# antofuller/jumbo_mae_tpu

Hardware: AMD Instinct MI355X
Metric: pretrain images/sec (whole node) ViT-L/16 224 mask75% at 1/2/4/8 MI355X (higher is better)
Workload: dtype bf16; 1 GPU; model=vit_large_patch16 jumbo-MAE (3 CLS, shared jumbo MLP) + decoder 8x512x16h, global_batch=4096, seq_len=52, decoder_seq_len=199, parallelism=dp1, per_gpu_batch=4096, grad_accum=2, micro_batch=2048, grad_ckpt=False, hip_graph=False, optimizer=adamw(0.9,0.95) wd0.05 warmup-cosine

## Files before the change

### jumbo_mae_tpu_amd/csrc/bindings.cpp

```cpp
#include <torch/extension.h>
#include <c10/hip/HIPStream.h>
#include <hip/hip_runtime.h>

#include <climits>

#include "jm_api.h"

namespace {

hipStream_t stream() { return c10::hip::getCurrentHIPStream().stream(); }

#define CHECK_CUDA(x) TORCH_CHECK((x).is_cuda(), #x " must be a GPU tensor")
#define CHECK_CONTIG(x) TORCH_CHECK((x).is_contiguous(), #x " must be contiguous")
#define CHECK_DT(x, d) TORCH_CHECK((x).scalar_type() == (d), #x " has wrong dtype")

const uint16_t* bf(const torch::Tensor& t) { return reinterpret_cast<const uint16_t*>(t.data_ptr()); }
uint16_t* bfm(torch::Tensor& t) { return reinterpret_cast<uint16_t*>(t.data_ptr()); }
uint16_t* bfp(const torch::Tensor& t) { return reinterpret_cast<uint16_t*>(t.data_ptr()); }
const float* fopt(const c10::optional<torch::Tensor>& t) {
  return t.has_value() && t->defined() ? t->data_ptr<float>() : nullptr;
}
float* fopt_m(c10::optional<torch::Tensor>& t) { return t.has_value() && t->defined() ? t->data_ptr<float>() : nullptr; }

void check_rc(int rc, const char* what) { TORCH_CHECK(rc == 0, what, ": unsupported shape (rc=", rc, ")"); }
// ... 2 lines not shown
  TORCH_CHECK(rate >= 0.0 && rate < 1.0, "dropout rate must be in [0, 1)");
  const double keep = 1.0 - rate;
  return {(uint32_t)std::llround(keep * 65536.0), (float)(1.0 / keep)};
}

static void check_seed(const torch::Tensor& seed, const torch::Tensor& like) {
  TORCH_CHECK(seed.scalar_type() == torch::kInt64 && seed.numel() == 1 && seed.device() == like.device(),
              "dropout seed: int64 [1] on the data's device");
}

JmDrop make_drop(const c10::optional<torch::Tensor>& seed, double rate, const torch::Tensor& like, int64_t ioff) {
  if (!seed.has_value() || !seed->defined() || rate <= 0.0) return JmDrop{nullptr, 0u, 1.f, 0};
  check_seed(*seed, like);
  const auto kp = keep_params(rate);
  return JmDrop{seed->data_ptr<int64_t>(), kp.first, kp.second, (long)ioff};
}

std::vector<torch::Tensor> layernorm_fwd(torch::Tensor x, torch::Tensor gamma, torch::Tensor beta, double eps,
                                         py::object out_dtype, bool also_bf16) {
  CHECK_CUDA(x);
  TORCH_CHECK(x.dim() == 3 && x.stride(2) == 1, "x must be [B,T,D] with contiguous last dim");
  CHECK_DT(x, torch::kFloat32);
  CHECK_CONTIG(gamma);
  CHECK_CONTIG(beta);
  const auto odt = torch::python::detail::py_object_to_dtype(out_dtype);
  const int B = x.size(0), T = x.size(1), D = x.size(2);
  auto y = torch::empty({(long)B * T, D}, x.options().dtype(odt));
  auto mean = torch::empty({(long)B * T}, x.options());
  auto rstd = torch::empty({(long)B * T}, x.options());
  TORCH_CHECK(odt == torch::kBFloat16 || odt == torch::kFloat32, "out dtype must be bf16/fp32");
// ... 74 lines not shown
    CHECK_CONTIG((*hx));
    TORCH_CHECK(hx->numel() == (long)B * T * D, "hx shape");
    TORCH_CHECK(beta.has_value() && beta->defined() && beta->numel() == D, "hx needs beta [D]");
    CHECK_DT((*beta), torch::kFloat32);
    hxp = bf(*hx);
    betap = beta->data_ptr<float>();
  }
  const int NP = has_res ? 4 : 2;
  auto ws = torch::empty({(accum || has_res) ? (long)jm_layernorm_bwd_blocks(B * T, D) * NP * D : 1}, x.options());
  check_rc(jm_layernorm_bwd(dy.data_ptr(), dyb, x.data_ptr<float>(), x.stride(0), x.stride(1), B, T, D,
                            mean.data_ptr<float>(), rstd.data_ptr<float>(), gamma.data_ptr<float>(),
                            dx.data_ptr<float>(), dx.stride(0), dx.stride(1), rp, rB, rT, dgamma.data_ptr<float>(),
                            dbeta.data_ptr<float>(), accum, ws.data_ptr<float>(), has_res ? &res : nullptr,
                            stream(), hxp, betap),
           "layernorm_bwd");
  if (has_res) return {dx, dyr};
  return {dx};
}

torch::Tensor gelu_fwd(torch::Tensor h) {
  CHECK_CONTIG(h);
  CHECK_DT(h, torch::kBFloat16);
  auto a = torch::empty_like(h);
  check_rc(jm_gelu_fwd(bf(h), bfm(a), h.numel(), stream()), "gelu_fwd");
  return a;
}

static torch::Tensor rowcol_ws(const torch::Tensor& like, int M, int N, int nacc) {
  const long n = jm_rowcol_ws_floats(M, N, nacc);
  return torch::empty({n > 0 ? n : 1}, like.options().dtype(torch::kFloat32));
}

torch::Tensor gelu_bwd(torch::Tensor h, torch::Tensor da, c10::optional<torch::Tensor> bias_grad, bool deriv) {
  CHECK_CONTIG(h);
  CHECK_CONTIG(da);
  CHECK_DT(h, torch::kBFloat16);
  CHECK_DT(da, torch::kBFloat16);
  const int N = h.size(-1);
  const int M = h.numel() / N;
  auto dh = torch::empty_like(h);
  float* bg = fopt_m(bias_grad);
  torch::Tensor ws;
  if (bg) ws = rowcol_ws(h, M, N, 1);
  check_rc(jm_gelu_bwd(bf(h), bf(da), bfm(dh), bg, M, N, stream(), deriv ? 1 : 0, bg ? ws.data_ptr<float>() : nullptr),
           "gelu_bwd");
  return dh;
}

void colsum(torch::Tensor x, torch::Tensor acc) {
  CHECK_CONTIG(x);
  CHECK_DT(x, torch::kBFloat16);
  const int N = x.size(-1);
  const int M = x.numel() / N;
  auto ws = rowcol_ws(x, M, N, 1);
  check_rc(jm_colsum_bf16(bf(x), acc.data_ptr<float>(), M, N, stream(), ws.data_ptr<float>()), "colsum");
}

void splitk_reduce_add(torch::Tensor part, torch::Tensor g) {
  CHECK_CONTIG(part);
  TORCH_CHECK(g.is_contiguous() && g.numel() * part.size(0) == part.numel(), "splitk_reduce_add shapes");
  check_rc(jm_splitk_reduce_add(part.data_ptr<float>(), g.data_ptr<float>(), g.numel(), part.size(0), stream()),
           "splitk_reduce_add");
}

void colsum_add_f32(torch::Tensor x, torch::Tensor g) {
  CHECK_CUDA(x);
  CHECK_DT(x, torch::kFloat32);
  CHECK_DT(g, torch::kFloat32);
  TORCH_CHECK(x.dim() == 2 && x.stride(1) == 1 && g.is_contiguous() && g.numel() == x.size(1),
              "colsum_add_f32: x [rows, n] with unit column stride, g [n]");
  TORCH_CHECK(reinterpret_cast<uintptr_t>(x.data_ptr()) % 16 == 0 && reinterpret_cast<uintptr_t>(g.data_ptr()) % 16 == 0,
              "colsum_add_f32: 16-byte aligned operands");
  check_rc(jm_colsum_add_f32(x.data_ptr<float>(), x.stride(0), x.size(0), x.size(1), g.data_ptr<float>(), stream()),
           "colsum_add_f32");
}

torch::Tensor residual_fwd(torch::Tensor x, torch::Tensor y, c10::optional<torch::Tensor> scale,
                           c10::optional<torch::Tensor> mask, c10::optional<torch::Tensor> out_opt,
                           c10::optional<torch::Tensor> seed, double rate, int64_t ioff) {
  TORCH_CHECK(x.dim() == 3 && x.stride(2) == 1, "x must be [B,T,D]");
  CHECK_DT(x, torch::kFloat32);
  CHECK_CONTIG(y);
  CHECK_DT(y, torch::kBFloat16);
  const int B = x.size(0), T = x.size(1), D = x.size(2);
  torch::Tensor out;
  if (out_opt.has_value() && out_opt->defined()) {
    out = *out_opt;
    TORCH_CHECK(out.dim() == 3 && out.size(0) == B && out.size(1) == T && out.size(2) == D && out.stride(2) == 1,
                "out view");
// ... 41 lines not shown
    } else {
      yB = oB;
      yT = oT;
    }
  } else {
    TORCH_CHECK(yB == (long)T * D && yT == D, "residual_bwd: a strided y needs out");
    dy = torch::empty({(long)B * T, D}, dout.options().dtype(odt));
  }
  torch::Tensor ws;
  const bool sums = (dscale && dscale->defined()) || (dbias && dbias->defined());
  if (sums) ws = rowcol_ws(dout, B * T, D, 2);
  check_rc(jm_residual_bwd(dout.data_ptr<float>(), dout.stride(0), dout.stride(1), has_y ? bf(*y) : nullptr,
                           fopt(scale), fopt(mask), fopt_m(dscale), bfm(dy), B, T, D, fopt_m(dbias), yB, yT,
                           stream(), make_drop(seed, rate, dout, ioff), sums ? ws.data_ptr<float>() : nullptr),
           "residual_bwd");
  return dy;
}

static std::tuple<const int64_t*, uint32_t, float> attn_drop(const c10::optional<torch::Tensor>& seed, double rate,
                                                             const torch::Tensor& like) {
  if (!seed.has_value() || !seed->defined() || rate <= 0.0) return {nullptr, 0u, 1.f};
  check_seed(*seed, like);
  const auto kp = keep_params(rate);
  return {seed->data_ptr<int64_t>(), kp.first, kp.second};
}

py::tuple attn_head_dims() {
  const int* d = nullptr;
  const int n = jm_attn_head_dims(&d);
  py::tuple t(n);
// ... 47 lines not shown
             "attn_bwd (long)");
    return dqkv;
  }
  torch::Tensor part;
  const int rows = jm_attn_bwd_part_rows(B, S, hd);
  if (dbias) {
    TORCH_CHECK(dbias->is_contiguous() && dbias->scalar_type() == torch::kFloat32 && dbias->numel() == D3,
                "attn_bwd: dbias must be contiguous fp32 [3D]");
    part = torch::empty({rows, D3}, qkv.options().dtype(torch::kFloat32));
  }
  float* pp = dbias ? part.data_ptr<float>() : nullptr;
  check_rc(jm_attn_bwd(bf(qkv), bf(o), bf(dO), lse.data_ptr<float>(), bfm(dqkv), B, S, heads, hd, pp, std::get<0>(dr),
                       std::get<1>(dr), std::get<2>(dr), stream()),
           "attn_bwd");
  if (dbias) check_rc(jm_splitk_reduce_add(pp, dbias->data_ptr<float>(), D3, rows, stream()), "attn_bwd dbias");
  return dqkv;
}

int nch(const torch::Tensor& chunks) { return chunks.size(0); }
const int* chp(const torch::Tensor& chunks) { return chunks.data_ptr<int>(); }
uint16_t* shadow_ptr(c10::optional<torch::Tensor>& s) {
  return (s.has_value() && s->defined()) ? reinterpret_cast<uint16_t*>(s->data_ptr()) : nullptr;
}

torch::Tensor chunk_part(const torch::Tensor& like, const torch::Tensor& chunks, int nc) {
  return torch::empty({(long)nch(chunks) * nc + 1}, like.options().dtype(torch::kFloat32));
}

void opt_sumsq(torch::Tensor x, torch::Tensor chunks, torch::Tensor out) {
  auto cp = chunk_part(x, chunks, 1);
// ... 322 lines not shown
  torch::Tensor ws;
  const int epi = deriv ? 7 : 2;
  const int r = attach_tail(ep, ws, M, N, K, epi, A);
  int nM = jm_gemm_nt_colpart_rows(M, N, K, epi, A.stride(0));
  if (dbias) {
    TORCH_CHECK(dbias->is_contiguous() && dbias->scalar_type() == torch::kFloat32 && dbias->numel() == N,
                "gemm_nt_dgelu dbias");
    part = r ? torch::zeros({nM + 8 * r, N}, A.options().dtype(torch::kFloat32))
             : torch::empty({nM, N}, A.options().dtype(torch::kFloat32));
    ep.colpart = part.data_ptr<float>();
    nM += 8 * r;
  }
  check_rc(jm_gemm_nt(bf(A), A.stride(0), bf(B), B.stride(0), M, N, K, epi, ep, stream()), "gemm_nt_dgelu");
  if (dbias) check_rc(jm_splitk_reduce_add(part.data_ptr<float>(), dbias->data_ptr<float>(), N, nM, stream()),
                      "gemm_nt_dgelu dbias");
  return out;
}

torch::Tensor rrc_resize(torch::Tensor src, torch::Tensor tab, int64_t size, int64_t tmp_bytes, int64_t tmp_rows_max) {
  CHECK_CUDA(src);
  CHECK_CUDA(tab);
  CHECK_DT(src, torch::kUInt8);
  CHECK_DT(tab, torch::kInt64);
  TORCH_CHECK(src.dim() == 1 && src.is_contiguous(), "rrc_resize: src must be a flat uint8 buffer");
  TORCH_CHECK(tab.dim() == 2 && tab.size(1) == 13 && tab.is_contiguous(), "rrc_resize: tab [B, 13] int64");
  TORCH_CHECK(size > 0 && size <= 4096 && tmp_bytes > 0 && tmp_rows_max > 0, "rrc_resize: bad sizes");
  const int B = tab.size(0);
  auto out = torch::empty({B, 3, size, size}, src.options());
  auto tmp = torch::empty({tmp_bytes}, src.options());
  check_rc(jm_rrc_resize(src.data_ptr<uint8_t>(), tab.data_ptr<int64_t>(), B, (int)size, tmp.data_ptr<uint8_t>(),
// ... 209 lines not shown
  const int sps = jm_gemm_tn_plan(grp, M, &S);
  torch::Tensor part;
  if (S > 1) part = torch::empty({S * total}, gs[0].options());
  int64_t off = 0;
  for (int p = 0; p < np; ++p) {
    grp.out[p] = S > 1 ? part.data_ptr<float>() + off : gs[p].data_ptr<float>();
    off += (int64_t)S * grp.N[p] * grp.K[p];
  }
  const int all_store = group_stores(stores, gs, S, np);
  check_rc(jm_gemm_tn(grp, segmented ? &segs : nullptr, M, sps, S, stream(), all_store), what);
  if (S > 1)
    for (int p = 0; p < np; ++p)
      check_rc(jm_splitk_reduce_add(grp.out[p], gs[p].data_ptr<float>(), (long)grp.N[p] * grp.K[p], S, stream(),
                                    p < (int)stores.size() && stores[p]),
               what);
  return S;
}

int64_t gemm_tn_wgrad(torch::Tensor dy, torch::Tensor x, torch::Tensor g, bool store) {
  return tn_wgrad("gemm_tn_wgrad", {Tensors{dy}}, {Tensors{x}}, {g}, {store}, false);
}

int64_t gemm_tn_wgrad_seg(Tensors dys, Tensors xs, torch::Tensor g, bool store) {
  return tn_wgrad("gemm_tn_wgrad_seg", {dys}, {xs}, {g}, {store}, true);
}

int64_t gemm_tn_wgrad_group(Tensors dys, Tensors xs, Tensors gs, std::vector<bool> stores) {
  std::vector<Tensors> d, x;
  for (const auto& t : dys) d.push_back({t});
  for (const auto& t : xs) x.push_back({t});
// ... 83 lines not shown
  m.def("dropout_apply", &dropout_apply);
  m.def("dropout_apply_", &dropout_apply_);
  m.def("rrc_resize", &rrc_resize, py::arg("src"), py::arg("tab"), py::arg("size"), py::arg("tmp_bytes"),
        py::arg("tmp_rows_max"));
  m.def("rrc_kmax", &jm_rrc_kmax);
  m.def("window_resize", &window_resize, py::arg("src"), py::arg("tab"), py::arg("size"), py::arg("tmp_bytes"),
        py::arg("tmp_rows_max"));
  m.def("window_tab", &jm_window_tab);
  m.def("aug_chain", &aug_chain, py::arg("images"), py::arg("chain"), py::arg("scratch"));
  m.def("gelu_drop", &gelu_drop, py::arg("a"), py::arg("b") = py::none(), py::arg("seed"), py::arg("rate"));
  m.def("softmax_dropout_fwd", &softmax_dropout_fwd);
  m.def("softmax_dropout_bwd", &softmax_dropout_bwd);
  m.def("gelu_bwd", &gelu_bwd, py::arg("h"), py::arg("da"), py::arg("bias_grad") = py::none(),
        py::arg("deriv") = false);
  m.def("colsum", &colsum);
  m.def("splitk_reduce_add", &splitk_reduce_add);
  m.def("residual_ln_fwd", &residual_ln_fwd, py::arg("x"), py::arg("y"), py::arg("scale"), py::arg("mask"),
        py::arg("gamma"), py::arg("beta"), py::arg("eps"), py::arg("T0"), py::arg("R0") = 0,
        py::arg("out") = py::none(), py::arg("seed") = py::none(), py::arg("rate") = 0.0);
  m.def("transpose_bf16", &transpose_bf16);
  m.def("residual_fwd", &residual_fwd, py::arg("x"), py::arg("y"), py::arg("scale"), py::arg("mask"),
        py::arg("out") = py::none(), py::arg("seed") = py::none(), py::arg("rate") = 0.0, py::arg("ioff") = 0);
  m.def("residual_bwd", &residual_bwd, py::arg("dout"), py::arg("y"), py::arg("scale"), py::arg("mask"),
        py::arg("dscale"), py::arg("ydtype"), py::arg("dbias") = py::none(), py::arg("out") = py::none(),
        py::arg("seed") = py::none(), py::arg("rate") = 0.0, py::arg("ioff") = 0);
  m.def("attn_fwd", &attn_fwd, py::arg("qkv"), py::arg("heads"), py::arg("seed") = py::none(), py::arg("rate") = 0.0);
  m.def("attn_bwd", &attn_bwd, py::arg("dO"), py::arg("qkv"), py::arg("o"), py::arg("lse"), py::arg("heads"),
        py::arg("dbias") = py::none(), py::arg("seed") = py::none(), py::arg("rate") = 0.0);
  m.def("attn_max_seq", &jm_attn_max_seq);
  m.def("attn_head_dims", &attn_head_dims);
  m.def("attn_fused_bias", &attn_fused_bias, py::arg("S"), py::arg("hd"));
// ... 58 lines not shown
```

### jumbo_mae_tpu_amd/csrc/elementwise.hip

```cpp
#include "common.h"
#include "jm_api.h"

namespace {

JM_DEVICE float gelu_f(float h) { return gelu_tanh_f(h); }
JM_DEVICE float gelu_grad(float h) { return gelu_grad_f(h); }

__global__ __launch_bounds__(256) void gelu_fwd_kernel(const uint16_t* __restrict__ h, uint16_t* __restrict__ a,
                                                       long n8) {
  for (long i = blockIdx.x * 256L + threadIdx.x; i < n8; i += (long)gridDim.x * 256) {
    float v[8];
    load8(h + i * 8, v);
#pragma unroll
    for (int j = 0; j < 8; ++j) v[j] = gelu_f(v[j]);
    store8(a + i * 8, v);
  }
}

struct ColPlan {
  int cgs, tpr, rps;
};

JM_DEVICE ColPlan col_plan(int N) {
  ColPlan p;
// ... 320 lines not shown
    }
    __syncthreads();
  }
  if (rl == 0 && i < n4) {
    float4* gp = reinterpret_cast<float4*>(g) + i;
    float4 o = store ? make_float4(0.f, 0.f, 0.f, 0.f) : *gp;
    const float4 r = red[c];
    o.x += r.x;
    o.y += r.y;
    o.z += r.z;
    o.w += r.w;
    *gp = o;
  }
}

void launch_colsum(const float* part, float* g, long n4, int S, long ld, int store, hipStream_t st) {
  const long blocks = (n4 + 255) / 256;
  if (blocks >= 512 || S < 16) {
    if (store) jm_zero_f32(g, n4 * 4, st);
    splitk_reduce_add_kernel<<<(unsigned)(blocks > 4096 ? 4096 : blocks), 256, 0, st>>>(part, g, n4, S, ld);
    return;
  }
  int rl = 16;
  while (rl < 256 && S > 32 * rl) rl *= 2;
  const unsigned nb = (unsigned)((n4 * rl + 255) / 256);
  switch (rl) {
    case 16: colsum_rows_kernel<16><<<nb, 256, 0, st>>>(part, g, n4, S, ld, store); break;
    case 32: colsum_rows_kernel<32><<<nb, 256, 0, st>>>(part, g, n4, S, ld, store); break;
    case 64: colsum_rows_kernel<64><<<nb, 256, 0, st>>>(part, g, n4, S, ld, store); break;
    case 128: colsum_rows_kernel<128><<<nb, 256, 0, st>>>(part, g, n4, S, ld, store); break;
    default: colsum_rows_kernel<256><<<nb, 256, 0, st>>>(part, g, n4, S, ld, store); break;
// ... 23 lines not shown
  for (long i = (long)blockIdx.x * 256 + threadIdx.x; i < n; i += (long)gridDim.x * 256) p[i] = 0.f;
}
}

void jm_zero_f32(float* p, long n, hipStream_t st) {
  if (n <= 0) return;
  long blocks = (n + 255) / 256;
  if (blocks > 2048) blocks = 2048;
  zero_f32_kernel<<<(unsigned)blocks, 256, 0, st>>>(p, n);
}

int jm_splitk_reduce_add(const float* part, float* g, long n, int S, hipStream_t st, int store) {
  if (n % 4) return -1;
  const long n4 = n / 4;
  if (S >= 1 && S <= 16 && n4 >= 256L * 256) {
    const unsigned nb = (unsigned)((n4 + 255) / 256);
    switch (S) {
#define JM_SKR(SS)                                                                     \
  case SS:                                                                             \
    if (store) splitk_reduce_add_s_kernel<SS, true><<<nb, 256, 0, st>>>(part, g, n4);  \
    else splitk_reduce_add_s_kernel<SS><<<nb, 256, 0, st>>>(part, g, n4);              \
    return 0;
      JM_SKR(1) JM_SKR(2) JM_SKR(3) JM_SKR(4) JM_SKR(5) JM_SKR(6) JM_SKR(7) JM_SKR(8)
      JM_SKR(9) JM_SKR(10) JM_SKR(11) JM_SKR(12) JM_SKR(13) JM_SKR(14) JM_SKR(15) JM_SKR(16)
#undef JM_SKR
      default: break;
    }
  }
  launch_colsum(part, g, n4, S, n, store, st);
  return 0;
}

int jm_colsum_add_f32(const float* x, long ld, int rows, long n, float* g, hipStream_t st) {
  if (n % 4 || ld % 4 || ld < n || rows < 1) return -1;
  launch_colsum(x, g, n / 4, rows, ld, 0, st);
  return 0;
}

namespace {
__global__ __launch_bounds__(256) void zero_ranges_kernel(float* __restrict__ base, const long long* __restrict__ desc,
                                                          int n) {
  long long b = blockIdx.x;
  int r = 0;
  for (; r < n; ++r) {
    const long long nb = (desc[2 * r + 1] + 4095) / 4096;
// ... 229 lines not shown
```

### jumbo_mae_tpu_amd/csrc/jm_api.h

```cpp
#pragma once
#include <cstddef>
#include <cstdint>

#include <hip/hip_runtime.h>

struct JmDrop {
  const int64_t* seed;
  uint32_t thr;
  float scale;
  long ioff;
};

struct JmLnRes {
  const uint16_t* y;
  uint16_t* dy;
  long yB, yT;
  const float* scale;
  const float* mask;
  int T0;
  float* dscale;
  float* dbias;
  JmDrop drop;
};

// ... 23 lines not shown
  float* colpart;
  float* part;
  int splits;
  float* tail;
  int tail_S;
  int t_begin;
  int t_count;
  const int64_t* dseed;
  uint32_t dthr;
  float dscale;
  uint8_t* dq;
  const uint8_t* dqa;
  float dqs;
};


int jm_layernorm_fwd(const float* x, long sB, long sT, int B, int T, int D, const float* gamma, const float* beta,
                     float eps, void* y, int out_bf16, float* mean, float* rstd, hipStream_t st, uint16_t* y2 = nullptr);
int jm_layernorm_bwd(const void* dy, int dy_bf16, const float* x, long sB, long sT, int B, int T, int D,
                     const float* mean, const float* rstd, const float* gamma, float* dx_ptr, long oB, long oT,
                     const float* dres, long rB, long rT, float* dgamma, float* dbeta, int accum_params, float* ws,
                     const JmLnRes* res, hipStream_t st, const uint16_t* hx = nullptr,
                     const float* beta = nullptr);
int jm_layernorm_bwd_blocks(int rows, int D);
int jm_residual_ln_fwd(const float* x, long sB, long sT, const uint16_t* y, const float* scale, const float* mask,
                       float* x1, long oB, long oT, uint16_t* h, float* mean, float* rstd, int B, int T, int T0,
                       int D, const float* gamma, const float* beta, float eps, hipStream_t st, int R0 = 0,
                       JmDrop drop = JmDrop{nullptr, 0u, 1.f, 0});
int jm_debug_line_layernorm();

int jm_gelu_fwd(const uint16_t* h, uint16_t* a, long n, hipStream_t st);
long jm_rowcol_ws_floats(int M, int N, int nacc);
int jm_gelu_bwd(const uint16_t* h, const uint16_t* da, uint16_t* dh, float* bias_grad, int M, int N, hipStream_t st,
                int deriv, float* ws);
int jm_colsum_bf16(const uint16_t* x, float* acc, int M, int N, hipStream_t st, float* ws);
int jm_residual_fwd(const float* x, long sB, long sT, int B, int T, int D, const uint16_t* y, const float* scale,
                    const float* mask, float* out, long oB, long oT, hipStream_t st, JmDrop drop);
int jm_residual_bwd(const float* dout, long dB, long dT, const uint16_t* y, const float* scale, const float* mask,
                    float* dscale, uint16_t* dy, int B, int T, int D, float* dbias, long yB, long yT, hipStream_t st,
                    JmDrop drop, float* ws);
void jm_zero_f32(float* p, long n, hipStream_t st);
int jm_splitk_reduce_add(const float* part, float* g, long n, int S, hipStream_t st, int store = 0);
int jm_colsum_add_f32(const float* x, long ld, int rows, long n, float* g, hipStream_t st);
int jm_zero_ranges(float* base, const long long* desc, int n, long long blocks, hipStream_t st);
int jm_transpose_bf16(const uint16_t* src, uint16_t* dst, int R, int C, hipStream_t st);
int jm_transpose_bf16_batch(const long long* desc, int n, int tiles, hipStream_t st);
int jm_splitk_reduce_bf16(const float* part, int S, long n, int N, const float* bias, uint16_t* out, hipStream_t st);
int jm_splitk_reduce_f32(const float* part, int S, int M, int N, const float* bias, const float* add, long add_ld,
                         float* out, hipStream_t st);
int jm_debug_line_elementwise();
void jm_debug_selftest(int v, hipStream_t st);

int jm_attn_fwd(const uint16_t* qkv, uint16_t* o, float* lse, int B, int S, int H, int hd, const int64_t* dseed,
                uint32_t dthr, float dscale, hipStream_t st);
int jm_attn_bwd(const uint16_t* qkv, const uint16_t* o, const uint16_t* dO, const float* lse, uint16_t* dqkv, int B,
                int S, int H, int hd, float* dbias_part, const int64_t* dseed, uint32_t dthr, float dscale,
                hipStream_t st);
// ... 83 lines not shown
```

### jumbo_mae_tpu_amd/csrc/layernorm.hip

```cpp
#include <type_traits>

#include "common.h"
#include "jm_api.h"

namespace {

template <int V, typename TO>
__global__ __launch_bounds__(256) void ln_fwd_kernel(const float* __restrict__ x, long sB, long sT, int T,
                                                     int rows, int D, const float* __restrict__ gamma,
                                                     const float* __restrict__ beta, float eps,
                                                     TO* __restrict__ y, float* __restrict__ mean_out,
                                                     float* __restrict__ rstd_out, uint16_t* __restrict__ y2) {
  const int wave = threadIdx.x >> 6, lane = threadIdx.x & 63;
  const int row = blockIdx.x * 4 + wave;
  if (row >= rows) return;
  const int b = row / T, t = row - b * T;
  const float* xr = x + b * sB + t * sT;
  float v[V][4];
  float s = 0.f;
#pragma unroll
  for (int i = 0; i < V; ++i) {
    const int col = (i * 64 + lane) * 4;
    if (col < D) {
      load4(xr + col, v[i]);
// ... 398 lines not shown
    __syncthreads();
  }
  if (rl == 0 && i4 < n4) {
    const float4 r = red[c];
    const float v[4] = {r.x, r.y, r.z, r.w};
#pragma unroll
    for (int j = 0; j < 4; ++j) {
      const int col = i4 * 4 + j;
      float* dst = outs.p[col / D];
      if (dst != nullptr) dst[col % D] += v[j];
    }
  }
}

void launch_param_reduce(const float* ws, int nb, int D, int NP, ParamOuts outs, hipStream_t st) {
  int rl = 16;
  while (rl < 256 && nb > 32 * rl) rl *= 2;
  const unsigned grid = (unsigned)((NP * D / 4) * rl + 255) / 256;
  switch (rl) {
    case 16: ln_param_reduce_kernel<16><<<grid, 256, 0, st>>>(ws, nb, D, NP, outs); break;
    case 32: ln_param_reduce_kernel<32><<<grid, 256, 0, st>>>(ws, nb, D, NP, outs); break;
    case 64: ln_param_reduce_kernel<64><<<grid, 256, 0, st>>>(ws, nb, D, NP, outs); break;
    case 128: ln_param_reduce_kernel<128><<<grid, 256, 0, st>>>(ws, nb, D, NP, outs); break;
    default: ln_param_reduce_kernel<256><<<grid, 256, 0, st>>>(ws, nb, D, NP, outs); break;
  }
}

template <typename TO>
void launch_fwd(int V, dim3 grid, hipStream_t st, const float* x, long sB, long sT, int T, int rows, int D,
                const float* g, const float* b, float eps, TO* y, float* m, float* r, uint16_t* y2) {
// ... 210 lines not shown
                       int D, const float* gamma, const float* beta, float eps, hipStream_t st, int R0,
                       JmDrop drop) {
  const ResLnIO io{x, sB, sT, y, scale, mask, x1, oB, oT, h, mean, rstd, drop};
  if (R0 < 0 || R0 >= T) return -2;
  const int V = pick_v(D);
  if (V < 0 || (D % 4) != 0) return -1;
  const int rows = B * T;
  dim3 grid((rows + 3) / 4);
#define JM_RLN(VV) \
  case VV: res_ln_fwd_kernel<VV><<<grid, 256, 0, st>>>(io, T, T0, R0, rows, D, gamma, beta, eps); break;
  switch (V) {
    JM_RLN(1) JM_RLN(2) JM_RLN(3) JM_RLN(4) JM_RLN(6) JM_RLN(8) JM_RLN(9) JM_RLN(12) JM_RLN(16)
    default: return -1;
  }
#undef JM_RLN
  return 0;
}

constexpr int LN_BWD_CUS = 256;
int ln_bwd_blocks_per_cu(int V) { return V <= 1 ? 4 : V <= 4 ? 3 : 2; }

int jm_layernorm_bwd_blocks(int rows, int D) {
  if (use_wide(rows, D)) return rows > 1024 ? 1024 : rows;
  const int V = pick_v(D), cap = LN_BWD_CUS * ln_bwd_blocks_per_cu(V < 0 ? 16 : V);
  const int rpb = 4 * LN_BWD_R(V);
  int nb = (rows + rpb - 1) / rpb;
  return nb > cap ? cap : nb;
}

int jm_layernorm_bwd(const void* dy, int dy_bf16, const float* x, long sB, long sT, int B, int T, int D,
// ... 65 lines not shown
```

### jumbo_mae_tpu_amd/ops/blocks.py

```python

from __future__ import annotations


import torch

from typing import NamedTuple

from . import dropout as Dr
from . import prims as P


LINKS = True
FWD_LINKS = True


class Link:

    __slots__ = ("spec", "dy", "done", "dx_key", "ln1", "h1")

    def __init__(self, ln1=None):
        self.spec = None
        self.dy = None
        self.done = False
        self.dx_key = None
# ... 107 lines not shown
        else:
            P.residual_fwd(pin, fy, layer.scale2, m2, out=x2[:, C:], drop=_od(dr, "fo", fy))
        ctx.save_for_backward(x, mu1, rs1, h1, qkv, o, lse, a, x1, muc, rsc, hcb, jpre, jg, jy,
                              hp, mup, rsp, fpre, fg, fy, m1, m2, m3)
        ctx.layer = layer
        ctx.link_in, ctx.link_out = link_in, link_out
        ctx.gelu_deriv = (jd, fd)
        ctx.gelu_rate = rate
        ctx.dr = dr
        if link_out is not None:
            link_out.spec = P.ResSpec(fy, layer.scale2, m2, layer.ff.w2.b, C, drop=_od(dr, "fo", fy))
        return x2

    @staticmethod
    def backward(ctx, dx2):
        with P.paired_wgrads():
            dx = _jumbo_bwd(ctx, dx2)
        return dx, None, None, None, None, None, None, None, None, None


def _jumbo_bwd(ctx, dx2):
    (x, mu1, rs1, h1, qkv, o, lse, a, x1, muc, rsc, hcb, jpre, jg, jy,
     hp, mup, rsp, fpre, fg, fy, m1, m2, m3) = ctx.saved_tensors
    layer = ctx.layer
    dr = ctx.dr
    B, S, D = x.shape
    C = layer.C
    J = C * D
    dt = h1.dtype
    dx2 = dx2.contiguous()
    dx1 = torch.empty_like(dx2)
# ... 66 lines not shown
            link_out.put_h1(x2, h1n, mun, rsn)
        else:
            x2 = P.residual_fwd(x1, fy, layer.scale2, m2, drop=_od(dr, "fo", fy))
        ctx.save_for_backward(x, mu1, rs1, h1, qkv, o, lse, a, x1, mu2, rs2, h2, fpre, fg, fy, m1, m2)
        ctx.layer = layer
        ctx.link_in, ctx.link_out = link_in, link_out
        ctx.gelu_deriv = (False, fd)
        ctx.gelu_rate = dr.rate if dr is not None else 0.0
        ctx.dr = dr
        if link_out is not None:
            link_out.spec = P.ResSpec(fy, layer.scale2, m2, layer.ff.w2.b, 0, drop=_od(dr, "fo", fy))
        return x2

    @staticmethod
    def backward(ctx, dx2):
        with P.paired_wgrads():
            dx = _vit_bwd(ctx, dx2)
        return dx, None, None, None, None, None, None, None, None


def _vit_bwd(ctx, dx2):
    x, mu1, rs1, h1, qkv, o, lse, a, x1, mu2, rs2, h2, fpre, fg, fy, m1, m2 = ctx.saved_tensors
    layer = ctx.layer
    dr = ctx.dr
    B, S, D = x.shape
    dt = h1.dtype
    dx2 = dx2.contiguous()
    fused = ctx.link_out.take(dx2) if ctx.link_out is not None else None
    if fused is not None:
        dfy, bd = fused
    else:
# ... 15 lines not shown
```

### jumbo_mae_tpu_amd/ops/prims.py

```python

from __future__ import annotations

import contextlib
import math
import os

from typing import NamedTuple

import torch
import torch.nn.functional as F

from ..models.params import Handle
from . import _ext

LN_EPS = 1e-6
_GELU_C = math.sqrt(2.0 / math.pi)


def hip(t: torch.Tensor) -> bool:
    return _ext.use_hip(t)


def _trainable(h: Handle | None) -> bool:
    return h is not None and h.segs[0].trainable
# ... 37 lines not shown
            part = torch.bmm(dy.view(s, M // s, N).transpose(1, 2), x.view(s, M // s, K), out_dtype=torch.float32)
            if hip(part):
                _ext.load().splitk_reduce_add(part, g)
            else:
                g.add_(part.sum(0))
        else:
            torch.addmm(g, dy.t(), x, out_dtype=torch.float32, out=g)
    else:
        g.addmm_(dy.t().float(), x.float())


PAIR_WGRAD = True
_pair: dict = {"depth": 0, "held": None}


@contextlib.contextmanager
def paired_wgrads():
    _pair["depth"] += 1
    try:
        yield
    finally:
        _pair["depth"] -= 1
        if _pair["depth"] == 0:
            _flush_pair()


def _flush_pair() -> None:
    held, _pair["held"] = _pair["held"], None
    if held is not None:
        hw, dy, x = held
        wgrad(hw, dy, x)
        hw.ready()


def _wgrad_ready(hw: Handle, dy: torch.Tensor, x: torch.Tensor) -> None:
    if PAIR_WGRAD and _pair["depth"] > 0 and _tn_ok(dy, x):
        held = _pair["held"]
        if held is not None and held[1].shape[0] == dy.shape[0] and held[0] is not hw:
            _pair["held"] = None
            _ext.load().gemm_tn_wgrad_group([held[1], dy], [held[2], x], [held[0].grad, hw.grad],
                                            [held[0].take_store(), hw.take_store()])
            held[0].ready()
            hw.ready()
            return
        _flush_pair()
        _pair["held"] = (hw, dy, x)
        return
    wgrad(hw, dy, x)
    hw.ready()


def bias_grad(hb: Handle, dy: torch.Tensor) -> None:
    if hip(dy) and dy.dtype == torch.bfloat16 and dy.shape[-1] % 8 == 0 and dy.stride(-1) == 1:
        _ext.load().colsum(dy, hb.grad)
    else:
        hb.grad.add_(dy.sum(0, dtype=torch.float32))


_GEMM_MODE = "auto"
_DGRAD_OURS = True


NARROW_MAX_M = 4096
_NARROW_FUSED_MIN_TILES = 160
# ... 117 lines not shown

def _flush_seg_group(todo: list) -> list:
    if not GROUP_JUMBO_WGRAD or len(todo) != 2:
        return todo
    (h1, p1), (h2, p2) = todo
    if any(h.store.partial_hooks and len(h.segs) == 1 for h in (h1, h2)) or len(p1) != len(p2):
        return todo
    d1, x1 = [p[0] for p in p1], [p[1] for p in p1]
    d2, x2 = [p[0] for p in p2], [p[1] for p in p2]
    if not (_seg_ok(d1, x1) and _seg_ok(d2, x2) and d1[0].shape[0] == d2[0].shape[0]
            and d1[0].shape[0] % 64 == 0 and h1.grad.is_contiguous() and h2.grad.is_contiguous()):
        return todo
    _ext.load().gemm_tn_wgrad_seg_group([d1, d2], [x1, x2], [h1.grad, h2.grad], [h1.take_store(), h2.take_store()])
    for h, pairs in todo:
        for _ in pairs:
            h.ready()
    return []


def flush_deferred_wgrads() -> None:
    _deferred["cb"] = False
    hs, _deferred["handles"] = _deferred["handles"], []
    todo = []
    for h in hs:
        pairs, h.deferred = h.deferred, []
        if pairs:
            todo.append((h, pairs))
    for h, pairs in _flush_seg_group(todo):
        dys = [p[0] for p in pairs]
        xs = [p[1] for p in pairs]
        N, K = dys[0].shape[1], xs[0].shape[1]
# ... 5 lines not shown
            dy = torch.cat(dys) if len(dys) > 1 else dys[0]
            x = torch.cat(xs) if len(xs) > 1 else xs[0]
        store = h.take_store() if seg else False
        if len(chunks) > 1 and not seg:
            h.settle()
        for r0, r1 in chunks:
            if seg:
                _ext.load().gemm_tn_wgrad_seg([d[:, r0:r1] for d in dys], xs, h.grad[r0:r1], store)
            elif len(chunks) == 1:
                wgrad(h, dy, x)
            else:
                wgrad(h, dy[:, r0:r1], x, rows=(r0, r1))
            if len(chunks) > 1:
                h.store.mark_partial_ready(h, r0 * K, r1 * K)
        for _ in pairs:
            h.ready()


def _defer_wgrad(hw: Handle, dy: torch.Tensor, x2: torch.Tensor) -> bool:
    if not _deferred["cb"]:
        try:
            torch.autograd.Variable._execution_engine.queue_callback(flush_deferred_wgrads)
        except RuntimeError:
            return False
        _deferred["cb"] = True
    if not hw.deferred:
        _deferred["handles"].append(hw)
    hw.deferred.append((dy, x2))
    return True


# ... 34 lines not shown
        return _ext.load().gemm_nt(dy.contiguous(), hw.weight_t(), None, False)[0]
    if (_DGRAD_OURS and hip(dy) and dy.dtype == torch.bfloat16 and w.shape[0] % 64
            and use_our_gemm(dy.shape[0], w.shape[1], -(-w.shape[0] // 64) * 64, kind="dgrad")):
        return _ext.load().gemm_nt(_pad_cols(dy), _pad_cols(hw.weight_t()), None, False)[0]
    return dy @ w


def linear_bwd(dy: torch.Tensor, x2: torch.Tensor, hw: Handle, hb: Handle | None, need_dx: bool = True,
               bias_done: bool = False, dx_add: torch.Tensor | None = None):
    dx = linear_dgrad(dy, hw, dx_add) if need_dx else None
    if (_trainable(hw) and hw.defer_wgrad and _deferred["enabled"] and (hip(dy) or _deferred["force"])
            and _defer_wgrad(hw, dy, x2)):
        if hb is not None:
            if not bias_done:
                bias_grad(hb, dy)
            hb.ready()
        return dx
    if _trainable(hw):
        side = wgrad_stream() if dy.is_cuda else None
        if side is not None:
            if not _side["cb"]:
                torch.autograd.Variable._execution_engine.queue_callback(_end_of_backward)
                _side["cb"] = True
            side.wait_stream(torch.cuda.current_stream())
            with torch.cuda.stream(side):
                wgrad(hw, dy, x2)
                if hb is not None and not bias_done:
                    bias_grad(hb, dy)
            dy.record_stream(side)
            x2.record_stream(side)
            hw.ready()
        else:
            if hb is not None and not bias_done:
                bias_grad(hb, dy)
            _wgrad_ready(hw, dy, x2)
        if hb is not None:
            hb.ready()
    return dx


def linear_gelu_bwd(dy: torch.Tensor, g: torch.Tensor, pre: torch.Tensor, hw2: Handle, hb2: Handle | None,
                    hb1: Handle | None, bias2_done: bool = False, deriv: bool = False, rate: float = 0.0):
    w2 = hw2.weight()
    M, N, K = dy.shape[0], w2.shape[1], w2.shape[0]
    if (_DGRAD_OURS and hip(dy) and dy.dtype == torch.bfloat16 and N % 8 == 0
            and (not deriv or pre.dtype == torch.uint8)
            and use_our_gemm(M, N, K, fused_gelu=True, kind="dgrad")):
        bg = hb1.grad if _trainable(hb1) else None
        dpre = _ext.load().gemm_nt_dgelu(dy.contiguous(), hw2.weight_t(), pre.contiguous(), bg, deriv, rate)
        linear_bwd(dy, g, hw2, hb2, need_dx=False, bias_done=bias2_done)
        return dpre, bg is not None
    if deriv and pre.dtype == torch.uint8:
# ... 93 lines not shown
        xf = x3.reshape(B * T, D).float()
        xhat = (xf - mean[:, None]) * rstd[:, None]
        dyf = dy.reshape(B * T, D).float()
        if tr:
            hg.grad.add_((dyf * xhat).sum(0))
            hb.grad.add_(dyf.sum(0))
        g = dyf * hg.master
        dx = rstd[:, None] * (g - g.mean(-1, keepdim=True) - xhat * (g * xhat).mean(-1, keepdim=True))
        dx = dx.reshape(B, T, D)
        if dres is not None:
            dx = dx + dres
        if out is not None:
            out.copy_(dx)
            dx = out
    if tr:
        hg.ready()
        hb.ready()
    if res is None:
        return dx
    if fused:
        if _trainable(res.hs):
            res.hs.ready()
        return dx, dyr, _trainable(res.hbias)
    dyr, done = residual_bwd(dx[:, res.t0:], res.y, res.hs, res.mask, res.y.dtype, res.hbias, out=res.out,
                             drop=res.drop)
    return dx, dyr, done


def residual_fwd(x3: torch.Tensor, y2: torch.Tensor, hs: Handle | None, mask, out=None, drop=None) -> torch.Tensor:
    B, T, D = x3.shape
    if hip(x3):
        y2r = y2.reshape(B * T, D)
        dseed, drate, dioff = _drop_args(y2r, drop)
        return _ext.load().residual_fwd(x3, y2r, hs.master if hs is not None else None, mask, out, dseed, drate,
                                        dioff)
    r = y2.float()
    if drop is not None:
# ... 45 lines not shown
            d = d * mask.view(B, 1, 1)
        if drop is not None:
            d = d * _drop_factor(y2, drop).reshape(B, T, D)
        if hs is not None:
            if _trainable(hs):
                hs.grad.add_((d * y2.float().reshape(B, T, D)).sum((0, 1)))
            d = d * hs.master
        dy = d.to(ydtype)
        if out is not None:
            out.copy_(dy.reshape(out.shape))
            dy = out
        else:
            dy = dy.reshape(B * T, D)
        done = False
    if mark_ready and _trainable(hs):
        hs.ready()
    return dy, done


def _attn_hip(qkv: torch.Tensor, heads: int) -> bool:
    if not hip(qkv):
        return False
    hd = qkv.shape[2] // 3 // heads
    return hd in _ext.load().attn_head_dims()


_ATTN_DROP_TILED = True


def _attn_drop_hip(S: int, hd: int) -> bool:
    ext = _ext.load()
# ... 57 lines not shown
```

Measured before the change: 6664 images/sec.

## Group small gradient reductions per block backward into one batched launch

Adds a grouped-reduction scope that queues the small parameter-gradient reductions issued during each transformer block's backward (LayerNorm param partials, bias colsums, split-K partial sums) and launches them together as one kernel with a job table, instead of one launch each. Workspaces are kept alive until the flush, and handle ready() calls are deferred until the group closes. The aim is to cut kernel-launch overhead and tail underutilisation from many tiny reductions. In exchange, gradient readiness for overlapping communication or optimizer work is delayed to the end of each block, and there is new bookkeeping for aliasing and stream consistency.

Result: no change. 6684 images/sec (median of 6 runs) (+0.3%).

```diff
diff --git a/jumbo_mae_tpu_amd/csrc/bindings.cpp b/jumbo_mae_tpu_amd/csrc/bindings.cpp
--- a/jumbo_mae_tpu_amd/csrc/bindings.cpp
+++ b/jumbo_mae_tpu_amd/csrc/bindings.cpp
@@ -40,6 +40,21 @@
   check_seed(*seed, like);
   const auto kp = keep_params(rate);
   return JmDrop{seed->data_ptr<int64_t>(), kp.first, kp.second, (long)ioff};
+}
+
+thread_local std::vector<torch::Tensor> rg_held;
+
+void rg_keep(const torch::Tensor& t) {
+  if (t.defined() && jm_rg_pending() > 0) rg_held.push_back(t);
+}
+
+void rg_begin(bool slices) { jm_rg_begin(slices ? 1 : 0); }
+
+int64_t rg_pending() { return jm_rg_pending(); }
+
+void rg_end() {
+  jm_rg_end(stream());
+  if (jm_rg_pending() == 0) rg_held.clear();
 }
 
 std::vector<torch::Tensor> layernorm_fwd(torch::Tensor x, torch::Tensor gamma, torch::Tensor beta, double eps,
@@ -144,6 +159,7 @@
                             dbeta.data_ptr<float>(), accum, ws.data_ptr<float>(), has_res ? &res : nullptr,
                             stream(), hxp, betap),
            "layernorm_bwd");
+  rg_keep(ws);
   if (has_res) return {dx, dyr};
   return {dx};
 }
@@ -174,6 +190,7 @@
   if (bg) ws = rowcol_ws(h, M, N, 1);
   check_rc(jm_gelu_bwd(bf(h), bf(da), bfm(dh), bg, M, N, stream(), deriv ? 1 : 0, bg ? ws.data_ptr<float>() : nullptr),
            "gelu_bwd");
+  rg_keep(ws);
   return dh;
 }
 
@@ -184,13 +201,35 @@
   const int M = x.numel() / N;
   auto ws = rowcol_ws(x, M, N, 1);
   check_rc(jm_colsum_bf16(bf(x), acc.data_ptr<float>(), M, N, stream(), ws.data_ptr<float>()), "colsum");
-}
-
-void splitk_reduce_add(torch::Tensor part, torch::Tensor g) {
+  rg_keep(ws);
+}
+
+void splitk_reduce_add(torch::Tensor part, torch::Tensor g, bool store) {
   CHECK_CONTIG(part);
   TORCH_CHECK(g.is_contiguous() && g.numel() * part.size(0) == part.numel(), "splitk_reduce_add shapes");
-  check_rc(jm_splitk_reduce_add(part.data_ptr<float>(), g.data_ptr<float>(), g.numel(), part.size(0), stream()),
+  check_rc(jm_splitk_reduce_add(part.data_ptr<float>(), g.data_ptr<float>(), g.numel(), part.size(0), stream(),
+                                store ? 1 : 0),
            "splitk_reduce_add");
+  rg_keep(part);
+}
+
+void ln_param_reduce(torch::Tensor ws, std::vector<c10::optional<torch::Tensor>> outs) {
+  CHECK_CUDA(ws);
+  CHECK_CONTIG(ws);
+  CHECK_DT(ws, torch::kFloat32);
+  const int NP = (int)outs.size();
+  TORCH_CHECK(ws.dim() == 2 && NP >= 1 && NP <= 4 && ws.size(1) % NP == 0, "ln_param_reduce: ws [nb, NP * D], NP <= 4");
+  const int D = ws.size(1) / NP;
+  float* po[4] = {nullptr, nullptr, nullptr, nullptr};
+  for (int k = 0; k < NP; ++k) {
+    if (!outs[k].has_value() || !outs[k]->defined()) continue;
+    TORCH_CHECK(outs[k]->is_contiguous() && outs[k]->scalar_type() == torch::kFloat32 && outs[k]->numel() == D &&
+                    outs[k]->device() == ws.device(),
+                "ln_param_reduce: outputs fp32 [D] on ws's device");
+    po[k] = outs[k]->data_ptr<float>();
+  }
+  check_rc(jm_ln_param_reduce(ws.data_ptr<float>(), (int)ws.size(0), D, NP, po, stream()), "ln_param_reduce");
+  rg_keep(ws);
 }
 
 void colsum_add_f32(torch::Tensor x, torch::Tensor g) {
@@ -203,6 +242,7 @@
               "colsum_add_f32: 16-byte aligned operands");
   check_rc(jm_colsum_add_f32(x.data_ptr<float>(), x.stride(0), x.size(0), x.size(1), g.data_ptr<float>(), stream()),
            "colsum_add_f32");
+  rg_keep(x);
 }
 
 torch::Tensor residual_fwd(torch::Tensor x, torch::Tensor y, c10::optional<torch::Tensor> scale,
@@ -274,6 +314,7 @@
                            fopt(scale), fopt(mask), fopt_m(dscale), bfm(dy), B, T, D, fopt_m(dbias), yB, yT,
                            stream(), make_drop(seed, rate, dout, ioff), sums ? ws.data_ptr<float>() : nullptr),
            "residual_bwd");
+  rg_keep(ws);
   return dy;
 }
 
@@ -351,6 +392,7 @@
                        std::get<1>(dr), std::get<2>(dr), stream()),
            "attn_bwd");
   if (dbias) check_rc(jm_splitk_reduce_add(pp, dbias->data_ptr<float>(), D3, rows, stream()), "attn_bwd dbias");
+  rg_keep(part);
   return dqkv;
 }
 
@@ -703,6 +745,7 @@
   check_rc(jm_gemm_nt(bf(A), A.stride(0), bf(B), B.stride(0), M, N, K, epi, ep, stream()), "gemm_nt_dgelu");
   if (dbias) check_rc(jm_splitk_reduce_add(part.data_ptr<float>(), dbias->data_ptr<float>(), N, nM, stream()),
                       "gemm_nt_dgelu dbias");
+  rg_keep(part);
   return out;
 }
 
@@ -942,6 +985,7 @@
       check_rc(jm_splitk_reduce_add(grp.out[p], gs[p].data_ptr<float>(), (long)grp.N[p] * grp.K[p], S, stream(),
                                     p < (int)stores.size() && stores[p]),
                what);
+  rg_keep(part);
   return S;
 }
 
@@ -1055,7 +1099,13 @@
   m.def("gelu_bwd", &gelu_bwd, py::arg("h"), py::arg("da"), py::arg("bias_grad") = py::none(),
         py::arg("deriv") = false);
   m.def("colsum", &colsum);
-  m.def("splitk_reduce_add", &splitk_reduce_add);
+  m.def("splitk_reduce_add", &splitk_reduce_add, py::arg("part"), py::arg("g"), py::arg("store") = false);
+  m.def("ln_param_reduce", &ln_param_reduce, "the LayerNorm backward's parameter-partial reduction alone");
+  m.def("rg_begin", &rg_begin, py::arg("slices") = false,
+        "open a grouped-reduction scope: the small gradient reductions issued until the matching rg_end run as one "
+        "launch there (slices: the weight gradients' split-K slice sums too)");
+  m.def("rg_end", &rg_end, "close the scope; the outermost one launches what is queued on the current stream");
+  m.def("rg_pending", &rg_pending, "queued reduction jobs");
   m.def("residual_ln_fwd", &residual_ln_fwd, py::arg("x"), py::arg("y"), py::arg("scale"), py::arg("mask"),
         py::arg("gamma"), py::arg("beta"), py::arg("eps"), py::arg("T0"), py::arg("R0") = 0,
         py::arg("out") = py::none(), py::arg("seed") = py::none(), py::arg("rate") = 0.0);
diff --git a/jumbo_mae_tpu_amd/csrc/elementwise.hip b/jumbo_mae_tpu_amd/csrc/elementwise.hip
--- a/jumbo_mae_tpu_amd/csrc/elementwise.hip
+++ b/jumbo_mae_tpu_amd/csrc/elementwise.hip
@@ -358,7 +358,181 @@
   }
 }
 
+namespace rg {
+__device__ __forceinline__ void rows_job(const RgJob& j, int lb, float4* red) {
+  const int RL = j.rl, CW = 256 / RL;
+  const int c = threadIdx.x % CW, rl = threadIdx.x / CW;
+  const long i = lb * (long)CW + c;
+  const int S = j.S;
+  float4 acc = make_float4(0.f, 0.f, 0.f, 0.f);
+  if (i < j.n4) {
+    const float4* p = reinterpret_cast<const float4*>(j.src) + i;
+    const long l4 = j.ld / 4;
+    int s = rl;
+    for (; s + 3 * RL < S; s += 4 * RL) {
+      const float4 a = p[(long)s * l4], b = p[(long)(s + RL) * l4];
+      const float4 e = p[(long)(s + 2 * RL) * l4], f = p[(long)(s + 3 * RL) * l4];
+      acc.x += (a.x + b.x) + (e.x + f.x);
+      acc.y += (a.y + b.y) + (e.y + f.y);
+      acc.z += (a.z + b.z) + (e.z + f.z);
+      acc.w += (a.w + b.w) + (e.w + f.w);
+    }
+    for (; s < S; s += RL) {
+      const float4 a = p[(long)s * l4];
+      acc.x += a.x;
+      acc.y += a.y;
+      acc.z += a.z;
+      acc.w += a.w;
+    }
+  }
+  red[threadIdx.x] = acc;
+  __syncthreads();
+  for (int h = RL / 2; h >= 1; h >>= 1) {
+    if (rl < h) {
+      const float4 o = red[threadIdx.x + h * CW];
+      float4& r = red[threadIdx.x];
+      r.x += o.x;
+      r.y += o.y;
+      r.z += o.z;
+      r.w += o.w;
+    }
+    __syncthreads();
+  }
+  if (rl == 0 && i < j.n4) {
+    float4* gp = reinterpret_cast<float4*>(j.dst) + i;
+    float4 o = j.store ? make_float4(0.f, 0.f, 0.f, 0.f) : *gp;
+    const float4 r = red[c];
+    o.x += r.x;
+    o.y += r.y;
+    o.z += r.z;
+    o.w += r.w;
+    *gp = o;
+  }
+}
+
+__device__ __forceinline__ void seq_job(const RgJob& j, int lb) {
+  const long i = lb * 256L + threadIdx.x;
+  if (i >= j.n4) return;
+  const long n = j.ld;
+  const int S = j.S;
+  float acc[4] = {0.f, 0.f, 0.f, 0.f};
+  int s = 0;
+  for (; s + 1 < S; s += 2) {
+    float v[4], w[4];
+    load4(j.src + (long)s * n + i * 4, v);
+    load4(j.src + (long)(s + 1) * n + i * 4, w);
+#pragma unroll
+    for (int k = 0; k < 4; ++k) acc[k] += v[k] + w[k];
+  }
+  if (s < S) {
+    float v[4];
+    load4(j.src + (long)s * n + i * 4, v);
+#pragma unroll
+    for (int k = 0; k < 4; ++k) acc[k] += v[k];
+  }
+  float o[4] = {0.f, 0.f, 0.f, 0.f};
+  if (!j.store) load4(j.dst + i * 4, o);
+#pragma unroll
+  for (int k = 0; k < 4; ++k) o[k] += acc[k];
+  store4(j.dst + i * 4, o);
+}
+
+__device__ __forceinline__ void slices_job(const RgJob& j, int lb) {
+  const long i = lb * 256L + threadIdx.x;
+  if (i >= j.n4) return;
+  const long n = j.ld;
+  const int S = j.S;
+  float o[4] = {0.f, 0.f, 0.f, 0.f};
+  if (!j.store) load4(j.dst + i * 4, o);
+  int s = 0;
+  for (; s + 3 < S; s += 4) {
+    float v[4][4];
+#pragma unroll
+    for (int u = 0; u < 4; ++u) load4(j.src + (long)(s + u) * n + i * 4, v[u]);
+#pragma unroll
+    for (int u = 0; u < 4; ++u)
+#pragma unroll
+      for (int k = 0; k < 4; ++k) o[k] += v[u][k];
+  }
+  for (; s < S; ++s) {
+    float v[4];
+    load4(j.src + (long)s * n + i * 4, v);
+#pragma unroll
+    for (int k = 0; k < 4; ++k) o[k] += v[k];
+  }
+  store4(j.dst + i * 4, o);
+}
+
+__global__ __launch_bounds__(256) void reduce_group_kernel(const RgTable tab) {
+  __shared__ float4 red[256];
+  const int b = blockIdx.x;
+  int lo = 0, hi = tab.n - 1;
+  while (lo < hi) {
+    const int mid = (lo + hi + 1) >> 1;
+    if (tab.job[mid].block0 <= b) lo = mid;
+    else hi = mid - 1;
+  }
+  const RgJob j = tab.job[lo];
+  const int lb = b - j.block0;
+  if (j.kind == RG_ROWS) rows_job(j, lb, red);
+  else if (j.kind == RG_SEQ) seq_job(j, lb);
+  else slices_job(j, lb);
+}
+
+struct Queue {
+  RgTable tab;
+  int depth = 0;
+  int slices = 0;
+  hipStream_t st = nullptr;
+};
+thread_local Queue q;
+
+void launch(hipStream_t st) {
+  if (q.tab.n == 0) return;
+  reduce_group_kernel<<<(unsigned)q.tab.blocks, 256, 0, st>>>(q.tab);
+  q.tab.n = 0;
+  q.tab.blocks = 0;
+}
+
+void push(RgJob j, long blocks, hipStream_t st) {
+  bool clash = q.tab.n == RG_MAX_JOBS || q.tab.blocks + blocks > (1L << 30);
+  for (int i = 0; i < q.tab.n && !clash; ++i) {
+    const RgJob& o = q.tab.job[i];
+    clash = j.dst < o.dst + o.n4 * 4 && o.dst < j.dst + j.n4 * 4;
+  }
+  if (clash) launch(q.st);
+  j.block0 = q.tab.blocks;
+  q.tab.job[q.tab.n++] = j;
+  q.tab.blocks += (int)blocks;
+  q.st = st;
+}
+
+bool open(hipStream_t st) { return q.depth > 0 && (q.tab.n == 0 || q.st == st); }
+
+bool aligned16(const void* p) { return reinterpret_cast<uintptr_t>(p) % 16 == 0; }
+
+int colsum_rl(int S) {
+  int rl = 16;
+  while (rl < 256 && S > 32 * rl) rl *= 2;
+  return rl;
+}
+
+void push_colsum(const float* part, float* g, long n4, int S, long ld, int store, bool rows, hipStream_t st) {
+  const long blocks = (n4 + 255) / 256;
+  if (!rows && (blocks >= 512 || S < 16)) {
+    push(RgJob{part, g, ld, n4, S, RG_SEQ, 0, store, 0}, blocks, st);
+    return;
+  }
+  const int rl = colsum_rl(S);
+  push(RgJob{part, g, ld, n4, S, RG_ROWS, rl, store, 0}, (n4 * rl + 255) / 256, st);
+}
+}
+
 void launch_colsum(const float* part, float* g, long n4, int S, long ld, int store, hipStream_t st) {
+  if (rg::open(st) && ld % 4 == 0 && rg::aligned16(part) && rg::aligned16(g)) {
+    rg::push_colsum(part, g, n4, S, ld, store, false, st);
+    return;
+  }
   const long blocks = (n4 + 255) / 256;
   if (blocks >= 512 || S < 16) {
     if (store) jm_zero_f32(g, n4 * 4, st);
@@ -412,6 +586,10 @@
   if (n % 4) return -1;
   const long n4 = n / 4;
   if (S >= 1 && S <= 16 && n4 >= 256L * 256) {
+    if (rg::q.slices && rg::open(st)) {
+      rg::push(RgJob{part, g, n, n4, S, RG_SLICES, 0, store, 0}, (n4 + 255) / 256, st);
+      return 0;
+    }
     const unsigned nb = (unsigned)((n4 + 255) / 256);
     switch (S) {
 #define JM_SKR(SS)                                                                     \
@@ -427,6 +605,27 @@
   }
   launch_colsum(part, g, n4, S, n, store, st);
   return 0;
+}
+
+void jm_rg_begin(int slices) {
+  if (rg::q.depth++ == 0) rg::q.slices = slices;
+}
+
+int jm_rg_pending() { return rg::q.tab.n; }
+
+void jm_rg_flush(hipStream_t st) { rg::launch(rg::q.tab.n ? rg::q.st : st); }
+
+void jm_rg_end(hipStream_t st) {
+  if (rg::q.depth > 0 && --rg::q.depth == 0) jm_rg_flush(st);
+}
+
+int jm_rg_ln_params(const float* ws, int nb, int D, int NP, float* const* outs, hipStream_t st) {
+  if (!rg::open(st) || D % 4 || !rg::aligned16(ws)) return 0;
+  for (int k = 0; k < NP; ++k)
+    if (outs[k] && !rg::aligned16(outs[k])) return 0;
+  for (int k = 0; k < NP; ++k)
+    if (outs[k]) rg::push_colsum(ws + (long)k * D, outs[k], D / 4, nb, (long)NP * D, 0, true, st);
+  return 1;
 }
 
 int jm_colsum_add_f32(const float* x, long ld, int rows, long n, float* g, hipStream_t st) {
diff --git a/jumbo_mae_tpu_amd/csrc/jm_api.h b/jumbo_mae_tpu_amd/csrc/jm_api.h
--- a/jumbo_mae_tpu_amd/csrc/jm_api.h
+++ b/jumbo_mae_tpu_amd/csrc/jm_api.h
@@ -61,6 +61,25 @@
   float dqs;
 };
 
+enum { RG_ROWS = 0, RG_SEQ = 1, RG_SLICES = 2 };
+struct RgJob {
+  const float* src;
+  float* dst;
+  long ld;
+  long n4;
+  int S;
+  int kind;
+  int rl;
+  int store;
+  int block0;
+};
+constexpr int RG_MAX_JOBS = 64;
+struct RgTable {
+  RgJob job[RG_MAX_JOBS];
+  int n;
+  int blocks;
+};
+
 
 int jm_layernorm_fwd(const float* x, long sB, long sT, int B, int T, int D, const float* gamma, const float* beta,
                      float eps, void* y, int out_bf16, float* mean, float* rstd, hipStream_t st, uint16_t* y2 = nullptr);
@@ -69,6 +88,7 @@
                      const float* dres, long rB, long rT, float* dgamma, float* dbeta, int accum_params, float* ws,
                      const JmLnRes* res, hipStream_t st, const uint16_t* hx = nullptr,
                      const float* beta = nullptr);
+int jm_ln_param_reduce(const float* ws, int nb, int D, int NP, float* const* outs, hipStream_t st);
 int jm_layernorm_bwd_blocks(int rows, int D);
 int jm_residual_ln_fwd(const float* x, long sB, long sT, const uint16_t* y, const float* scale, const float* mask,
                        float* x1, long oB, long oT, uint16_t* h, float* mean, float* rstd, int B, int T, int T0,
@@ -88,6 +108,11 @@
                     JmDrop drop, float* ws);
 void jm_zero_f32(float* p, long n, hipStream_t st);
 int jm_splitk_reduce_add(const float* part, float* g, long n, int S, hipStream_t st, int store = 0);
+void jm_rg_begin(int slices);
+void jm_rg_end(hipStream_t st);
+void jm_rg_flush(hipStream_t st);
+int jm_rg_pending();
+int jm_rg_ln_params(const float* ws, int nb, int D, int NP, float* const* outs, hipStream_t st);
 int jm_colsum_add_f32(const float* x, long ld, int rows, long n, float* g, hipStream_t st);
 int jm_zero_ranges(float* base, const long long* desc, int n, long long blocks, hipStream_t st);
 int jm_transpose_bf16(const uint16_t* src, uint16_t* dst, int R, int C, hipStream_t st);
diff --git a/jumbo_mae_tpu_amd/csrc/layernorm.hip b/jumbo_mae_tpu_amd/csrc/layernorm.hip
--- a/jumbo_mae_tpu_amd/csrc/layernorm.hip
+++ b/jumbo_mae_tpu_amd/csrc/layernorm.hip
@@ -436,6 +436,7 @@
 }
 
 void launch_param_reduce(const float* ws, int nb, int D, int NP, ParamOuts outs, hipStream_t st) {
+  if (jm_rg_ln_params(ws, nb, D, NP, outs.p, st)) return;
   int rl = 16;
   while (rl < 256 && nb > 32 * rl) rl *= 2;
   const unsigned grid = (unsigned)((NP * D / 4) * rl + 255) / 256;
@@ -676,6 +677,14 @@
     default: return -1;
   }
 #undef JM_RLN
+  return 0;
+}
+
+int jm_ln_param_reduce(const float* ws, int nb, int D, int NP, float* const* outs, hipStream_t st) {
+  if (D % 4 || NP < 1 || NP > 4 || nb < 1) return -1;
+  ParamOuts po{{nullptr, nullptr, nullptr, nullptr}};
+  for (int k = 0; k < NP; ++k) po.p[k] = outs[k];
+  launch_param_reduce(ws, nb, D, NP, po, st);
   return 0;
 }
 
diff --git a/jumbo_mae_tpu_amd/ops/blocks.py b/jumbo_mae_tpu_amd/ops/blocks.py
--- a/jumbo_mae_tpu_amd/ops/blocks.py
+++ b/jumbo_mae_tpu_amd/ops/blocks.py
@@ -145,7 +145,7 @@
 
     @staticmethod
     def backward(ctx, dx2):
-        with P.paired_wgrads():
+        with P.paired_wgrads(P.hip(dx2)):
             dx = _jumbo_bwd(ctx, dx2)
         return dx, None, None, None, None, None, None, None, None, None
 
@@ -242,7 +242,7 @@
 
     @staticmethod
     def backward(ctx, dx2):
-        with P.paired_wgrads():
+        with P.paired_wgrads(P.hip(dx2)):
             dx = _vit_bwd(ctx, dx2)
         return dx, None, None, None, None, None, None, None, None
 
diff --git a/jumbo_mae_tpu_amd/ops/prims.py b/jumbo_mae_tpu_amd/ops/prims.py
--- a/jumbo_mae_tpu_amd/ops/prims.py
+++ b/jumbo_mae_tpu_amd/ops/prims.py
@@ -75,15 +75,43 @@
 _pair: dict = {"depth": 0, "held": None}
 
 
+GROUP_REDUCE = os.environ.get("JMAE_GROUP_REDUCE", "1") != "0"
+GROUP_SLICES = False
+_group: dict = {"on": False, "ready": []}
+
+
+def _ready(h: Handle) -> None:
+    if _group["on"]:
+        _group["ready"].append(h)
+    else:
+        h.ready()
+
+
+def _group_end() -> None:
+    _group["on"] = False
+    hs, _group["ready"] = _group["ready"], []
+    _ext.load().rg_end()
+    for h in hs:
+        h.ready()
+
+
 @contextlib.contextmanager
-def paired_wgrads():
+def paired_wgrads(group: bool = False):
     _pair["depth"] += 1
+    opened = group and GROUP_REDUCE and not _group["on"]
+    if opened:
+        _ext.load().rg_begin(GROUP_SLICES)
+        _group["on"] = True
     try:
         yield
     finally:
         _pair["depth"] -= 1
-        if _pair["depth"] == 0:
-            _flush_pair()
+        try:
+            if _pair["depth"] == 0:
+                _flush_pair()
+        finally:
+            if opened:
+                _group_end()
 
 
 def _flush_pair() -> None:
@@ -91,7 +119,7 @@
     if held is not None:
         hw, dy, x = held
         wgrad(hw, dy, x)
-        hw.ready()
+        _ready(hw)
 
 
 def _wgrad_ready(hw: Handle, dy: torch.Tensor, x: torch.Tensor) -> None:
@@ -101,14 +129,14 @@
             _pair["held"] = None
             _ext.load().gemm_tn_wgrad_group([held[1], dy], [held[2], x], [held[0].grad, hw.grad],
                                             [held[0].take_store(), hw.take_store()])
-            held[0].ready()
-            hw.ready()
+            _ready(held[0])
+            _ready(hw)
             return
         _flush_pair()
         _pair["held"] = (hw, dy, x)
         return
     wgrad(hw, dy, x)
-    hw.ready()
+    _ready(hw)
 
 
 def bias_grad(hb: Handle, dy: torch.Tensor) -> None:
@@ -256,7 +284,7 @@
     _ext.load().gemm_tn_wgrad_seg_group([d1, d2], [x1, x2], [h1.grad, h2.grad], [h1.take_store(), h2.take_store()])
     for h, pairs in todo:
         for _ in pairs:
-            h.ready()
+            _ready(h)
     return []
 
 
@@ -292,7 +320,7 @@
             if len(chunks) > 1:
                 h.store.mark_partial_ready(h, r0 * K, r1 * K)
         for _ in pairs:
-            h.ready()
+            _ready(h)
 
 
 def _defer_wgrad(hw: Handle, dy: torch.Tensor, x2: torch.Tensor) -> bool:
@@ -357,7 +385,7 @@
         if hb is not None:
             if not bias_done:
                 bias_grad(hb, dy)
-            hb.ready()
+            _ready(hb)
         return dx
     if _trainable(hw):
         side = wgrad_stream() if dy.is_cuda else None
@@ -372,13 +400,13 @@
                     bias_grad(hb, dy)
             dy.record_stream(side)
             x2.record_stream(side)
-            hw.ready()
+            _ready(hw)
         else:
             if hb is not None and not bias_done:
                 bias_grad(hb, dy)
             _wgrad_ready(hw, dy, x2)
         if hb is not None:
-            hb.ready()
+            _ready(hb)
     return dx
 
 
@@ -502,13 +530,13 @@
             out.copy_(dx)
             dx = out
     if tr:
-        hg.ready()
-        hb.ready()
+        _ready(hg)
+        _ready(hb)
     if res is None:
         return dx
     if fused:
         if _trainable(res.hs):
-            res.hs.ready()
+            _ready(res.hs)
         return dx, dyr, _trainable(res.hbias)
     dyr, done = residual_bwd(dx[:, res.t0:], res.y, res.hs, res.mask, res.y.dtype, res.hbias, out=res.out,
                              drop=res.drop)
@@ -584,7 +612,7 @@
             dy = dy.reshape(B * T, D)
         done = False
     if mark_ready and _trainable(hs):
-        hs.ready()
+        _ready(hs)
     return dy, done
 
 
```
